# adityamwagh/SuperSLAM

Measured on AMD Instinct MI355X. Metric: stereo pairs/sec (SPx2+LG) at 1376x376, higher is better.
Workload: dtype f16; 1 GPU; configs[1]: SuperPoint x2 + select + gather + 1x LightGlue on 1376x376 stereo pairs; a step = 8 x 64 = 512 pairs per GPU resident in HBM (8 library calls of 64 pairs, different images per call), max_keypoints 600, seeded synthetic weights; pairs_per_call=64, max_keypoints=600, matches_last_call=1412, parallelism=replicated weights, pairs sharded over 1 rank(s), no data-path collective

## Files before the change

superslam_amd/csrc/lg_ffn.h:

```cpp
#pragma once
#include "igemm.h"
#include "kernels.h"

namespace sship {

constexpr int kFfnLd = 520;
typedef float f2_t __attribute__((ext_vector_type(2)));
constexpr float kGeluQ0 = -2.301893292e+00f, kGeluQ1 = -1.054467824e-01f, kGeluQ2 = 4.423903354e-04f, kGeluQ3 = 7.747288073e-05f,
                kGeluQ4 = -2.787147429e-06f;
__device__ __forceinline__ f2_t gelu2(f2_t y) {
  const f2_t s = y * y;
  f2_t q = s * kGeluQ4 + kGeluQ3;
  q = q * s + kGeluQ2;
  q = q * s + kGeluQ1;
  q = q * s + kGeluQ0;
  const f2_t t = y * q;
  const f2_t d = {1.0f + __builtin_amdgcn_exp2f(t[0]), 1.0f + __builtin_amdgcn_exp2f(t[1])};
  const f2_t r = {__builtin_amdgcn_rcpf(d[0]), __builtin_amdgcn_rcpf(d[1])};
  return y * r;
}
struct FfnTail {
  int ntiles;
  IgemmArgs proj;
  unsigned long long* trace;
  int trace_it;
  const float* match_w;
  float match_b;
  float* logsig;
  int n_main;
  const void* pf_ptr[3];
  int pf_bytes[3];
  const int* live;
  int tiles_per_pair;
};

bool ffn16_applicable(int tokens, int next_mt, bool heads);
hipError_t launch_lg_ffn16(int tokens, int next_mt, bool heads, hipStream_t s, const _Float16* ctx, const _Float16* w0p, const float* b0,
                           const float* gamma, const float* beta, const _Float16* w3p, const float* b3, _Float16* x, FfnTail t);

}
```

superslam_amd/csrc/lg_kernels.hip:

```cpp
#include <cstdlib>
#include <type_traits>

#include "igemm.h"
#include "kernels.h"
#include "lg_ffn.h"

namespace sship {

__global__ __launch_bounds__(256) void k_lg_prep(const float* __restrict__ kp, int kp_stride, int kp_seq_stride,
                                                 const int* __restrict__ lens, int max_kp, int* __restrict__ lens_clamped,
                                                 const _Float16* __restrict__ desc,
                                                 size_t desc_seq_stride, const float* __restrict__ wr, float img_w,
                                                 float img_h, int S, int NP, _Float16* __restrict__ x,
                                                 float* __restrict__ rope, float* __restrict__ kpn) {
  if (blockIdx.x == 0 && (int)threadIdx.x < S) lens_clamped[threadIdx.x] = min(max(lens[threadIdx.x], 0), max_kp);
  if (blockIdx.x == 0)
    for (int i = 256 + threadIdx.x; i < S; i += 256) lens_clamped[i] = min(max(lens[i], 0), max_kp);
  const int token = blockIdx.x * 4 + (threadIdx.x >> 6);
  const int lane = threadIdx.x & 63;
  if (token >= S * NP) return;
  const int s = token / NP, n = token % NP;
  const bool valid = n < min(max(lens[s], 0), max_kp);
  h4_t v = to_h4(0.f, 0.f, 0.f, 0.f);
  if (valid) v = *reinterpret_cast<const h4_t*>(desc + (size_t)s * desc_seq_stride + (size_t)n * 256 + lane * 4);
// ... 421 lines not shown
  } else {
    launch_attn<1, 4>(q, k, vt, lens, d, cross, ctx, s);
  }
}

#ifndef SSHIP_FFN_ABL
#define SSHIP_FFN_ABL 0
#endif
#ifndef SSHIP_FFN_DEEP_PFK
#define SSHIP_FFN_DEEP_PFK 4
#endif
#ifndef SSHIP_FFN_DEEP
#define SSHIP_FFN_DEEP 1
#endif
__device__ __forceinline__ void ffn_bar_lds() { asm volatile("s_waitcnt lgkmcnt(0)\n\ts_barrier" ::: "memory"); }
template <int AD>
__device__ __forceinline__ int ffn_live_tiles(const FfnTail& t) {
  if constexpr (AD == 1) return t.live[0] * t.tiles_per_pair;
  else if constexpr (AD == 2) return t.live[0];
  else return t.ntiles;
}
template <int AD>
__device__ __forceinline__ int ffn_tile_of(const FfnTail& t, int li) {
  if constexpr (AD == 1) return t.live[1 + li / t.tiles_per_pair] * t.tiles_per_pair + li % t.tiles_per_pair;
  else if constexpr (AD == 2) return t.live[1 + li];
  else return li;
}
template <int NEXT_MT, bool HEADS, int NT, bool PROJ, int AD = 0>
__global__ __launch_bounds__(512, 2) void k_lg_ffn(const _Float16* __restrict__ ctx, const _Float16* __restrict__ w0p,
                                                const float* __restrict__ b0, const float* __restrict__ gamma,
                                                const float* __restrict__ beta, const _Float16* __restrict__ w3p,
                                                const float* __restrict__ b3, _Float16* __restrict__ x, FfnTail tail) {
  constexpr int NTOK = NT * 32;
  constexpr bool DEEP = NT == 1 && !PROJ && SSHIP_FFN_DEEP;
  auto barrier = [&]() __attribute__((always_inline)) { if constexpr (DEEP) ffn_bar_lds(); else __syncthreads(); };
  constexpr int G0 = 4;
  constexpr int XBUF = NTOK * kFfnLd;
  extern __shared__ __attribute__((aligned(16))) char ffn_smem[];
  _Float16* s_xbuf = reinterpret_cast<_Float16*>(ffn_smem);
  float (*s_red)[NTOK] = reinterpret_cast<float (*)[NTOK]>(s_xbuf + (NT <= 2 ? 2 : 1) * XBUF);
  float* s_par = reinterpret_cast<float*>(s_red) + 16 * NTOK;
  for (int i = threadIdx.x; i < (PROJ ? 0 : 1792); i += 512)
    s_par[i] = i < 512 ? b0[i] : i < 1024 ? gamma[i - 512] : i < 1536 ? beta[i - 1024] : b3[i - 1536];
// ... 237 lines not shown
      const int rope_segs_t = pj.flags & 0xf;
      float4 cs[4][NT], bqk[NQK > 0 ? NQK : 1][4];
      if constexpr (HEADS) {
        if (rope_segs_t > 0) {
#pragma unroll
          for (int g = 0; g < 4; ++g)
#pragma unroll
            for (int n = 0; n < NT; ++n)
              cs[g][n] = *reinterpret_cast<const float4*>(pj.aux + (t0 + n * 32 + j) * 64 + ((wave * 32) & 63) + hh * 4 + g * 8 + zero);
        }
#pragma unroll
        for (int m = 0; m < NQK; ++m)
#pragma unroll
          for (int g = 0; g < 4; ++g) bqk[m][g] = *reinterpret_cast<const float4*>(pj.bias + (m * 8 + wave) * 32 + hh * 4 + g * 8);
      }
      constexpr int NG = (16 - PFK) / GT;
      h8_t at[2][GT][NEXT_MT];
      if constexpr (NG > 0) {
#pragma unroll
        for (int i = 0; i < GT; ++i)
#pragma unroll
          for (int m = 0; m < NEXT_MT; ++m) at[0][i][m] = *reinterpret_cast<const h8_t*>(wp + ((PFK + i) * NEXT_MT + m) * 512);
      }
      auto kstep = [&](int ks, const h8_t (&a)[NEXT_MT]) __attribute__((always_inline)) {
        h8_t bf[NT];
#pragma unroll
        for (int n = 0; n < NT; ++n) bf[n] = *reinterpret_cast<const h8_t*>(bfp + n * 32 * kFfnLd + ks * 16);
#pragma unroll
        for (int m = 0; m < NEXT_MT; ++m) {
#pragma unroll
// ... 71 lines not shown
                }
                const h2_t p01 = {(_Float16)v0, (_Float16)v1}, p23 = {(_Float16)v2, (_Float16)v3};
                lo[g] = __builtin_bit_cast(unsigned, p01);
                hi[g] = __builtin_bit_cast(unsigned, p23);
              }
#pragma unroll
              for (int gp = 0; gp < 2; ++gp) {
                const auto s0 = __builtin_amdgcn_permlane32_swap(lo[2 * gp], lo[2 * gp + 1], false, false);
                const auto s1 = __builtin_amdgcn_permlane32_swap(hi[2 * gp], hi[2 * gp + 1], false, false);
                const int u = ((R0 & 63) >> 3) + 2 * gp + hh;
                *reinterpret_cast<uint4*>(dst + (u >> 1) * 512 + (((u & 1) << 5) + j) * 8) = make_uint4(s0[0], s1[0], s0[1], s1[1]);
              }
            }
          }
        }
      } else {
        EpiF16<false, false>::template run<NEXT_MT, NT>(pj, ac3, 0, (int)(t0 >> 5), j, wave * NEXT_MT * 32, hh);
      }
    };
    if constexpr (HEADS) run_tail(std::integral_constant<int, 1 << (NEXT_MT - 1)>{});
    else run_tail(std::integral_constant<int, 0>{});
    if (tail.logsig) {
#pragma unroll 1
      for (int tk = wave * (NTOK / 8); tk < (wave + 1) * (NTOK / 8); ++tk) {
        const h4_t v = *reinterpret_cast<const h4_t*>(s_x + tk * kFfnLd + lane * 4);
        float d = 0.f;
#pragma unroll
        for (int e = 0; e < 4; ++e) d += (float)v[e] * mwq[lane * 4 + e];
        const float z = wave_sum(d) + tail.match_b;
        if (lane == 0) tail.logsig[t0 + tk] = fminf(z, 0.f) - log1pf(expf(-fabsf(z)));
      }
    }
  }
  stamp(9);
  if (NT > 2 && has_next) {
    __syncthreads();
    stage_tile(ffn_tile_of<AD>(tail, li + nwg), s_xn, wave, lane);
    asm volatile("s_waitcnt vmcnt(0)" ::: "memory");
  }
  if constexpr (PROJ) asm volatile("s_waitcnt vmcnt(0)" ::: "memory");
  if (has_next) __syncthreads();
  stamp(10);
  }
}
template <int NEXT_MT, bool HEADS, int NT, bool PROJ, int AD = 0, typename... A>
static hipError_t launch_ffn_nt(int tokens, int extra_wg, hipStream_t s, A... args) {
  constexpr size_t smem = (size_t)(NT <= 2 ? 2 : 1) * NT * 32 * kFfnLd * 2 + 16 * NT * 32 * 4 + 1792 * 4;
  static_assert(smem <= 163840, "LDS budget");
  auto kern = k_lg_ffn<NEXT_MT, HEADS, NT, PROJ, AD>;
  static const hipError_t attr_rc = hipFuncSetAttribute(reinterpret_cast<const void*>(kern), hipFuncAttributeMaxDynamicSharedMemorySize, (int)smem);
  if (attr_rc != hipSuccess) return attr_rc;
  const int ntiles = tokens / (NT * 32);
  hipLaunchKernelGGL(kern, dim3((ntiles < cu_count() ? ntiles : cu_count()) + extra_wg), dim3(512), smem, s, args...);
  return hipGetLastError();
}
static void ffn_trace_report(unsigned long long* dev, int nwg, int next_mt, hipStream_t s) {
  std::vector<unsigned long long> h((size_t)nwg * 8 * 12);
  (void)hipStreamSynchronize(s);
  (void)hipMemcpy(h.data(), dev, h.size() * 8, hipMemcpyDeviceToHost);
  static const char* names[10] = {"ffn.0", "LN stats", "DMA issue+GELU", "barrier", "ffn.3", "vmcnt+barrier+residual", "barrier", "tail MFMA", "tail epilogue", "end barrier"};
  double sum[10] = {0}; long cnt = 0;
  for (int w = 0; w < nwg * 8; ++w) {
    const unsigned long long* t = h.data() + (size_t)w * 12;
    if (!t[0] || !t[10]) continue;
    for (int i = 0; i < 10; ++i) sum[i] += (double)(t[i + 1] > t[i] ? t[i + 1] - t[i] : 0);
    ++cnt;
  }
  if (!cnt) return;
  fprintf(stderr, "[ffn trace next_mt=%d, %ld waves]", next_mt, cnt);
  double tot = 0;
  for (int i = 0; i < 10; ++i) { fprintf(stderr, " %s=%.0f", names[i], sum[i] / cnt); tot += sum[i] / cnt; }
  fprintf(stderr, " | tile=%.0f clk\n", tot);
}
template <int NEXT_MT, bool HEADS, int AD = 0, typename... A>
static hipError_t launch_ffn(int nt, int tokens, int extra_wg, hipStream_t s, A... args) {
  return nt == 1 ? launch_ffn_nt<NEXT_MT, HEADS, 1, false, AD>(tokens, extra_wg, s, args...)
                 : launch_ffn_nt<NEXT_MT, HEADS, 2, false, AD>(tokens, extra_wg, s, args...);
}
#ifndef SSHIP_FFN4_XROWS
#define SSHIP_FFN4_XROWS 1
#endif
#ifndef SSHIP_FFN4_BSTORE
#define SSHIP_FFN4_BSTORE 5
#endif
#ifndef SSHIP_FFN4_ABL
#define SSHIP_FFN4_ABL 0
#endif
__device__ __forceinline__ f16x_t mfma32_abl(h8_t a, h8_t b, f16x_t c) {
  if constexpr ((SSHIP_FFN4_ABL & 1) != 0) {
    asm volatile("" :: "v"(a), "v"(b));
    return c;
  } else {
    return mfma32(a, b, c);
  }
}
template <int NEXT_MT, bool HEADS, bool PROJ, int AD = 0>
__global__ __launch_bounds__(256, 2) void k_lg_ffn4(const _Float16* __restrict__ ctx, const _Float16* __restrict__ w0p,
                                                    const float* __restrict__ b0, const float* __restrict__ gamma,
                                                    const float* __restrict__ beta, const _Float16* __restrict__ w3p,
                                                    const float* __restrict__ b3, _Float16* __restrict__ x, FfnTail tail) {
  constexpr int NT = 2, NTOK = 64;
  extern __shared__ __attribute__((aligned(16))) char ffn_smem[];
  _Float16* s_x = reinterpret_cast<_Float16*>(ffn_smem);
  float (*s_red)[NTOK] = reinterpret_cast<float (*)[NTOK]>(s_x + NTOK * kFfnLd);
  float* s_par = reinterpret_cast<float*>(s_red) + 8 * NTOK;
  float* s_pb = s_par + 1792;
  float* s_b0b = s_pb + 768;
  for (int i = threadIdx.x; i < (PROJ ? 0 : 1792); i += 256)
    s_par[i] = i < 512 ? b0[i] : i < 1024 ? gamma[i - 512] : i < 1536 ? beta[i - 1024] : b3[i - 1536];
  for (int i = threadIdx.x; i < (PROJ ? 0 : 512); i += 256) s_b0b[i] = b0[i];
  if constexpr (NEXT_MT > 0 && HEADS)
    for (int i = threadIdx.x; i < NEXT_MT * 256; i += 256) s_pb[i] = tail.proj.bias[i];
  auto stage_tile = [&](int tile, int wave, int lane) {
    const size_t tt = (size_t)tile * NTOK;
    const char* gsrc = reinterpret_cast<const char*>((lane < 32 ? x + lane * 8 : ctx + (lane - 32) * 8) + (tt + wave) * 256);
#pragma unroll
    for (int k = 0; k < NTOK / 4; k += 2) {
      const unsigned lds0 = __builtin_amdgcn_readfirstlane((unsigned)(uintptr_t)(s_x + (wave + 4 * k) * kFfnLd));
      const unsigned lds1 = __builtin_amdgcn_readfirstlane((unsigned)(uintptr_t)(s_x + (wave + 4 * k + 4) * kFfnLd)) - 2048u;
      unsigned keep;
      asm volatile("s_mov_b32 %0, m0\n\ts_mov_b32 m0, %2\n\ts_nop 0\n\tglobal_load_lds_dwordx4 %1, off\n\t"
                   "s_mov_b32 m0, %3\n\ts_nop 0\n\tglobal_load_lds_dwordx4 %1, off offset:2048\n\ts_mov_b32 m0, %0"
                   : "=&s"(keep) : "v"(gsrc), "s"(lds0), "s"(lds1) : "memory");
      gsrc += 4096;
    }
  };
// ... 208 lines not shown
  stamp(6);
  }
  if constexpr (NEXT_MT > 0) {
    __syncthreads();
    stamp(7);
    if constexpr (SSHIP_FFN4_XROWS && !PROJ) {
#pragma unroll
      for (int r2 = 0; r2 < NTOK / 8; ++r2) {
        const int row = wave * (NTOK / 4) + 2 * r2 + hh;
        const uint4 u = *reinterpret_cast<const uint4*>(s_x + row * kFfnLd + j * 8);
        *reinterpret_cast<uint4*>(x + (t0 + row) * 256 + j * 8) = u;
      }
    }
    const int NP = pj.np, nt32 = NP >> 5;
    const int rope_segs = pj.flags & 0xf;
#pragma unroll 1
    for (int pass = 0; pass < 2; ++pass) {
      const int cb = wave + 4 * pass;
      f16x_t ac3[NEXT_MT][NT];
#pragma unroll
      for (int m = 0; m < NEXT_MT; ++m)
#pragma unroll
        for (int n = 0; n < NT; ++n)
#pragma unroll
          for (int r = 0; r < 16; ++r) ac3[m][n][r] = 0.f;
      float4 cs[4][NT];
      const __amdgpu_buffer_rsrc_t rrope = __builtin_amdgcn_make_buffer_rsrc(const_cast<float*>(tail.proj.aux), 0, (int)0x7ffffff0, 0x00020000);
      if constexpr (HEADS) {
        if (rope_segs > 0) {
#pragma unroll
// ... 92 lines not shown
                hi[g] = __builtin_bit_cast(unsigned, p23);
              }
#pragma unroll
              for (int gp = 0; gp < 2; ++gp) {
                const auto s0 = __builtin_amdgcn_permlane32_swap(lo[2 * gp], lo[2 * gp + 1], false, false);
                const auto s1 = __builtin_amdgcn_permlane32_swap(hi[2 * gp], hi[2 * gp + 1], false, false);
                if (SSHIP_FFN4_BSTORE & 4) wstore(rqk, lane16, dst + ((((R0 & 63) >> 3) + 2 * gp) >> 1) * 512, wq_t{s0[0], s1[0], s0[1], s1[1]});
                else {
                  const int u = ((R0 & 63) >> 3) + 2 * gp + hh;
                  *reinterpret_cast<uint4*>(static_cast<_Float16*>(seg == 0 ? pj.out0 : pj.out1) + dst + (u >> 1) * 512 + (((u & 1) << 5) + j) * 8) = make_uint4(s0[0], s1[0], s0[1], s1[1]);
                }
              }
            }
          }
        }
      } else {
        EpiF16<false, false>::template run<NEXT_MT, NT>(pj, ac3, 0, (int)(t0 >> 5), j, cb * NEXT_MT * 32, hh);
      }
    }
    if (tail.logsig) {
#pragma unroll 1
      for (int tk = wave * (NTOK / 4); tk < (wave + 1) * (NTOK / 4); ++tk) {
        const h4_t v = *reinterpret_cast<const h4_t*>(s_x + tk * kFfnLd + lane * 4);
        float d = 0.f;
#pragma unroll
        for (int e = 0; e < 4; ++e) d += (float)v[e] * mwq[lane * 4 + e];
        const float z = wave_sum(d) + tail.match_b;
        if (lane == 0) tail.logsig[t0 + tk] = fminf(z, 0.f) - log1pf(expf(-fabsf(z)));
      }
    }
  }
  stamp(10);
  if (has_next) {
    __syncthreads();
    stage_tile(ffn_tile_of<AD>(tail, li + (int)gridDim.x), wave, lane);
    asm volatile("s_waitcnt vmcnt(0)" ::: "memory");
    __syncthreads();
  }
  stamp(11);
  }
}
template <int NEXT_MT, bool HEADS, bool PROJ, int AD = 0, typename... A>
static hipError_t launch_ffn4(int tokens, hipStream_t s, A... args) {
  constexpr size_t smem = (size_t)64 * kFfnLd * 2 + 8 * 64 * 4 + (1792 + 768 + 512) * 4;
  static_assert(2 * smem <= 163840, "two workgroups must fit the CU's LDS");
  auto kern = k_lg_ffn4<NEXT_MT, HEADS, PROJ, AD>;
  static const hipError_t attr_rc = hipFuncSetAttribute(reinterpret_cast<const void*>(kern), hipFuncAttributeMaxDynamicSharedMemorySize, (int)smem);
  if (attr_rc != hipSuccess) return attr_rc;
  const int ntiles = tokens / 64;
  hipLaunchKernelGGL(kern, dim3(ntiles < 2 * cu_count() ? ntiles : 2 * cu_count()), dim3(256), smem, s, args...);
  return hipGetLastError();
}
static bool use_ffn4(int tokens) {
  static const int env = dev_env("SUPERSLAM_HIP_FFN") ? atoi(dev_env("SUPERSLAM_HIP_FFN")) : 0;
  if ((size_t)tokens * 512 >= 0x7f000000ull) return false;
  if (env == 8) return false;
  if (env == 4) return tokens % 64 == 0;
  return tokens % 64 == 0 && tokens / 64 >= 2 * cu_count();
}

[[maybe_unused]] static bool use_ffn16(int tokens) {
// ... 72 lines not shown
#if SSHIP_DEV_SWITCHES
  if (!live && use_ffn16(tokens) && ffn16_applicable(tokens, mt, heads)) {
    (void)launch_lg_ffn16(tokens, mt, heads, s, ctx, w0.w, w0.bias, gamma, beta, w3.w, w3.bias, x, t);
    return;
  }
#endif
  t.live = live;
  const int ad = live ? live_mode : 0;
  if (use_ffn4(tokens) && !trace_on_is8()) {
    t.ntiles = tokens / 64;
    t.tiles_per_pair = 2 * d.NP / 64;
    auto go4 = [&](auto ad_c) {
      constexpr int AD = decltype(ad_c)::value;
      if (heads && mt == 3) (void)launch_ffn4<3, true, false, AD>(tokens, s, ctx, w0.w, w0.bias, gamma, beta, w3.w, w3.bias, x, t);
      else if (heads && mt == 2) (void)launch_ffn4<2, true, false, AD>(tokens, s, ctx, w0.w, w0.bias, gamma, beta, w3.w, w3.bias, x, t);
      else (void)launch_ffn4<1, false, false, AD>(tokens, s, ctx, w0.w, w0.bias, gamma, beta, w3.w, w3.bias, x, t);
    };
    if (ad == 2) go4(std::integral_constant<int, 2>{});
    else if (ad == 1) go4(std::integral_constant<int, 1>{});
    else go4(std::integral_constant<int, 0>{});
    if (trace_on) ffn4_trace_report(trace_buf, t.ntiles < 2 * cu_count() ? t.ntiles : 2 * cu_count(), mt, s);
    return;
  }
  t.tiles_per_pair = 2 * d.NP / (nt * 32);
  const int extra = ffn_prefetch_setup(t, trace_wg, prefetch);
  auto go = [&](auto ad_c) {
    constexpr int AD = decltype(ad_c)::value;
    if (heads && mt == 3) (void)launch_ffn<3, true, AD>(nt, tokens, extra, s, ctx, w0.w, w0.bias, gamma, beta, w3.w, w3.bias, x, t);
    else if (heads && mt == 2) (void)launch_ffn<2, true, AD>(nt, tokens, extra, s, ctx, w0.w, w0.bias, gamma, beta, w3.w, w3.bias, x, t);
    else (void)launch_ffn<1, false, AD>(nt, tokens, extra, s, ctx, w0.w, w0.bias, gamma, beta, w3.w, w3.bias, x, t);
  };
  if (ad == 2) go(std::integral_constant<int, 2>{});
  else if (ad == 1) go(std::integral_constant<int, 1>{});
  else go(std::integral_constant<int, 0>{});
  if (trace_on) ffn_trace_report(trace_buf, trace_wg, mt, s);
}

hipError_t launch_lg_proj_heads(const ConvW& next, _Float16* x, LgDims d, int rope_segs, int t_seg, const float* rope, _Float16* q,
                                _Float16* k, _Float16* vt, hipStream_t s, const ConvW* const* prefetch, const int* tiles) {
  if (next.cout != 768) return hipErrorInvalidValue;
  const int tokens = d.S * d.NP;
  FfnTail t{};
  const int nt = tokens / 64 < cu_count() / 2 ? 1 : 2;
  t.ntiles = tokens / (nt * 32);
// ... 153 lines not shown
    ms = mutual ? expf(w[2 * NP + i]) : 0.f;
    mj = (mutual && ms > thr) ? j : -1;
  }
  matches0[(size_t)pair * max_kp + i] = mj;
  mscores0[(size_t)pair * max_kp + i] = ms;
}
#endif
constexpr float kLog2e = 1.44269504088896340736f;
__device__ __forceinline__ float fast_exp(float x) { return __builtin_amdgcn_exp2f(x * kLog2e); }
__device__ __forceinline__ void lse_merge(float& m, float& s, float m2, float s2) {
  const float M = fmaxf(m, m2);
  const float a = m > -INFINITY ? s * fast_exp(m - M) : 0.f, b = m2 > -INFINITY ? s2 * fast_exp(m2 - M) : 0.f;
  m = M; s = a + b;
}
constexpr int kAssignCh = 4;
__device__ __forceinline__ float fold_lse(const float2* p, int nparts, int NP) {
  float m = -INFINITY, s = 0.f;
  for (int k = 0; k < nparts; ++k) { const float2 v = p[(size_t)k * NP]; lse_merge(m, s, v.x, v.y); }
  return m + logf(s);
}
__device__ __forceinline__ void fold_argmax(const float2* p, int nparts, int NP, float& best, int& bi) {
  best = -INFINITY; bi = 0x7fffffff;
  for (int k = 0; k < nparts; ++k) {
    const float2 v = p[(size_t)k * NP];
    const int i = __float_as_int(v.y);
    if (v.x > best || (v.x == best && i < bi)) { best = v.x; bi = i; }
  }
}
template <int PASS>
__global__ __launch_bounds__(256, 2) void k_assign_stream(const _Float16* __restrict__ md, const float* __restrict__ logsig,
                                                       const int* __restrict__ lens, int NP, float* __restrict__ pcol,
                                                       float* __restrict__ prow, const float* __restrict__ pcol_in,
                                                       const float* __restrict__ prow_in) {
  constexpr int kChunkCols = (kMaxKp / 32 + kAssignCh - 1) / kAssignCh * 32;
  __shared__ __attribute__((aligned(16))) float s_lc[PASS ? kChunkCols : 4];
  __shared__ float s_lr[PASS ? 128 : 4];
  const int pair = blockIdx.y, wave = threadIdx.x >> 6, lane = threadIdx.x & 63, jl = lane & 31, hh = lane >> 5;
  const int NT = NP >> 5, ti = blockIdx.x * 4 + wave, i0 = ti * 32;
  const int n0 = min(max(lens[2 * pair], 0), NP), n1 = min(max(lens[2 * pair + 1], 0), NP);
  if ((int)blockIdx.x * 128 >= n0) return;
  const bool active = ti < NT && i0 < n0;
  const _Float16* A = md + ((size_t)(2 * pair) * NP + min(i0 + jl, NP - 1)) * 256 + hh * 8;
  const _Float16* Bm = md + (size_t)(2 * pair + 1) * NP * 256;
  h8_t fa[16];
#pragma unroll
  for (int ks = 0; ks < 16; ++ks) fa[ks] = *reinterpret_cast<const h8_t*>(A + ks * 16);
  const int my_i = i0 + jl;
  const int ro = 4 * hh;
  float c_i = 0.f, c_r[PASS ? 16 : 1];
  float rm = -INFINITY, rs = 0.f;
  int rj = 0x7fffffff;
  const int ntj_all = (n1 + 31) >> 5, per = (ntj_all + kAssignCh - 1) / kAssignCh;
  const int tj_lo = blockIdx.z * per, ntj = min(tj_lo + per, ntj_all);
  if (tj_lo >= ntj) return;
  const int jc0 = tj_lo * 32;
  if constexpr (PASS == 1) {
    const int nch = (ntj_all + per - 1) / max(per, 1), nrt = (n0 + 31) >> 5;
    if (threadIdx.x < 128) {
      const int i = blockIdx.x * 128 + threadIdx.x;
      s_lr[threadIdx.x] = i < n0 ? fold_lse(reinterpret_cast<const float2*>(prow_in) + (size_t)pair * kAssignCh * NP + i, nch, NP) : 0.f;
    }
    for (int j = threadIdx.x; j < (ntj - tj_lo) * 32; j += 256) {
      const int jj = jc0 + j;
      s_lc[j] = jj < n1 ? logsig[(size_t)(2 * pair + 1) * NP + jj] - fold_lse(reinterpret_cast<const float2*>(pcol_in) + (size_t)pair * NT * NP + jj, nrt, NP)
                        : 0.f;
    }
    __syncthreads();
    c_i = logsig[(size_t)(2 * pair) * NP + min(my_i, NP - 1)] - s_lr[wave * 32 + jl];
#pragma unroll
    for (int r = 0; r < 16; ++r) {
      const int il = (r & 3) + 8 * (r >> 2) + ro;
      c_r[r] = logsig[(size_t)(2 * pair) * NP + min(i0 + il, NP - 1)] - s_lr[wave * 32 + il];
    }
  }
  constexpr int kRowH = 264;
  __shared__ __attribute__((aligned(16))) _Float16 s_b[2][32 * kRowH];
  typedef unsigned stg_t __attribute__((ext_vector_type(4)));
  stg_t stg[4];
  auto fetch = [&](int tj) __attribute__((always_inline)) {
#pragma unroll
    for (int q = 0; q < 4; ++q) {
      const int u = threadIdx.x + 256 * q, row = u >> 5, unit = u & 31;
      stg[q] = *reinterpret_cast<const stg_t*>(Bm + (size_t)min(tj * 32 + row, NP - 1) * 256 + unit * 8);
    }
  };
  auto put = [&](int buf) __attribute__((always_inline)) {
#pragma unroll
    for (int q = 0; q < 4; ++q) {
      const int u = threadIdx.x + 256 * q, row = u >> 5, unit = u & 31;
      *reinterpret_cast<stg_t*>(&s_b[buf][row * kRowH + unit * 8]) = stg[q];
    }
  };
  fetch(tj_lo);
  put(0);
  __syncthreads();
  for (int tj = tj_lo; tj < ntj; ++tj) {
    const int j0 = tj * 32, buf = (tj - tj_lo) & 1;
    fetch(min(tj + 1, ntj - 1));
    const f16x_t zero16 = {0.f, 0.f, 0.f, 0.f, 0.f, 0.f, 0.f, 0.f, 0.f, 0.f, 0.f, 0.f, 0.f, 0.f, 0.f, 0.f};
    f16x_t ai = zero16, aj = zero16;
    if (active) {
      const _Float16* bt = &s_b[buf][jl * kRowH + hh * 8];
#pragma unroll
      for (int k = 0; k < 16; ++k) {
        const h8_t fbk = *reinterpret_cast<const h8_t*>(bt + k * 16);
        ai = mfma32(fbk, fa[k], ai);
        aj = mfma32(fa[k], fbk, aj);
// ... 45 lines not shown
#pragma unroll
      for (int g = 0; g < 4; ++g) {
        const int jb = j0 + 8 * g + ro;
        const float4 d4 = *reinterpret_cast<const float4*>(s_lc + jb - jc0);
        const float dv[4] = {d4.x, d4.y, d4.z, d4.w};
#pragma unroll
        for (int e = 0; e < 4; ++e) {
          const float v = fmaf(2.f, ai[4 * g + e], dv[e]);
          if (v > rm) { rm = v; rj = jb + e; }
        }
      }
      const float d_j = s_lc[my_j - jc0];
      float cv = -INFINITY;
      int ci = 0x7fffffff;
#pragma unroll
      for (int r = 0; r < 16; ++r) {
        const int i = i0 + (r & 3) + 8 * (r >> 2) + ro;
        const float v = fmaf(2.f, aj[r], c_r[r]);
        if (v > cv) { cv = v; ci = i; }
      }
      const float ov = __shfl_xor(cv, 32, 64);
      const int oi = __shfl_xor(ci, 32, 64);
      if (ov > cv || (ov == cv && oi < ci)) { cv = ov; ci = oi; }
      if (hh == 0 && my_j < n1)
        *reinterpret_cast<float2*>(pcol + (((size_t)pair * NT + ti) * NP + my_j) * 2) = make_float2(cv + d_j, __int_as_float(ci));
    }
  }
  float2* pr = reinterpret_cast<float2*>(prow) + ((size_t)pair * kAssignCh + blockIdx.z) * NP + my_i;
  if constexpr (PASS == 0) {
    lse_merge(rm, rs, __shfl_xor(rm, 32, 64), __shfl_xor(rs, 32, 64));
    if (hh == 0 && my_i < n0) *pr = make_float2(rm, rs);
  } else {
    const float ov = __shfl_xor(rm, 32, 64);
    const int oj = __shfl_xor(rj, 32, 64);
    if (ov > rm || (ov == rm && oj < rj)) { rm = ov; rj = oj; }
    if (hh == 0 && my_i < n0) *pr = make_float2(rm + c_i, __int_as_float(rj));
  }
}
__global__ __launch_bounds__(256) void k_assign_mutual(const float* __restrict__ pcol, const float* __restrict__ prow,
                                                       const int* __restrict__ lens, int NP, int max_kp, float thr,
                                                       int32_t* __restrict__ matches0, float* __restrict__ mscores0) {
  const int pair = blockIdx.y, i = blockIdx.x * blockDim.x + threadIdx.x;
  if (i >= max_kp) return;
  const int n0 = min(max(lens[2 * pair], 0), NP), n1 = min(max(lens[2 * pair + 1], 0), NP);
  const int NT = NP >> 5;
  int mj = -1;
  float ms = 0.f;
  if (i < n0 && n1 > 0) {
    const int ntj_all = (n1 + 31) >> 5, per = (ntj_all + kAssignCh - 1) / kAssignCh;
    float best, cbest;
    int j, ci;
    fold_argmax(reinterpret_cast<const float2*>(prow) + (size_t)pair * kAssignCh * NP + i, (ntj_all + per - 1) / max(per, 1), NP, best, j);
    if (j == 0x7fffffff) j = 0;
    bool mutual = false;
    if ((unsigned)j < (unsigned)n1) {
      fold_argmax(reinterpret_cast<const float2*>(pcol) + (size_t)pair * NT * NP + j, (n0 + 31) >> 5, NP, cbest, ci);
      mutual = (ci == 0x7fffffff ? 0 : ci) == i;
    }
    ms = mutual ? expf(best) : 0.f;
    mj = (mutual && ms > thr) ? j : -1;
  }
  matches0[(size_t)pair * max_kp + i] = mj;
  mscores0[(size_t)pair * max_kp + i] = ms;
}

void launch_lg_assign(const _Float16* md, const float* logsig, const int* lens, LgDims d, float* ws, float* pcol, int max_kp,
                      int32_t* matches0, float* mscores0, float thr, int stage, hipStream_t s) {
  const int P = d.S / 2, NT = d.NP / 32;
#if SSHIP_DEV_SWITCHES
  static const bool legacy = dev_env("SUPERSLAM_HIP_LG_ASSIGN") && std::string(dev_env("SUPERSLAM_HIP_LG_ASSIGN")) == "matrix";
  if (legacy && stage == 0) {
    float* sim = pcol;
    launch_lg_sim(md, lens, d, sim, s);
    hipLaunchKernelGGL(k_assign_row_lse, dim3(d.NP / 4, P), dim3(256), 0, s, sim, lens, d.NP, ws);
    hipLaunchKernelGGL(k_assign_col_lse, dim3((d.NP + 63) / 64, P), dim3(64 * kColRG), 0, s, sim, lens, d.NP, ws);
    hipLaunchKernelGGL(k_assign_row_arg, dim3(d.NP / 4, P), dim3(256), 0, s, sim, logsig, lens, d.NP, ws);
    hipLaunchKernelGGL(k_assign_col_arg, dim3((d.NP + 63) / 64, P), dim3(64 * kColRG), 0, s, sim, logsig, lens, d.NP, ws);
    hipLaunchKernelGGL(k_assign_final, dim3((max_kp + 255) / 256, P), dim3(256), 0, s, lens, d.NP, ws, max_kp, thr, matches0, mscores0);
    return;
  }
#endif
  {
    float* prow = pcol + (size_t)P * NT * d.NP * 2;
    float* pcol1 = prow + (size_t)P * kAssignCh * d.NP * 2;
    float* prow1 = pcol1 + (size_t)P * NT * d.NP * 2;
    if (stage == 0 || stage == 1)
      hipLaunchKernelGGL(k_assign_stream<0>, dim3((NT + 3) / 4, P, kAssignCh), dim3(256), 0, s, md, logsig, lens, d.NP, pcol, prow, nullptr, nullptr);
    if (stage == 0 || stage == 2)
      hipLaunchKernelGGL(k_assign_stream<1>, dim3((NT + 3) / 4, P, kAssignCh), dim3(256), 0, s, md, logsig, lens, d.NP, pcol1, prow1, pcol, prow);
    if (stage == 0)
      hipLaunchKernelGGL(k_assign_mutual, dim3((max_kp + 255) / 256, P), dim3(256), 0, s, pcol1, prow1, lens, d.NP, max_kp, thr, matches0, mscores0);
  }
}

__global__ __launch_bounds__(256) void k_lg_depth_init(const int* __restrict__ lens, int np, LgDepth dep) {
  for (int q = threadIdx.x; q < np; q += 256) {
    dep.layers_run[q] = 9;
#pragma unroll
    for (int i = 0; i < 8; ++i) dep.cnt[q * 8 + i] = 0;
    dep.lens_live[2 * q] = lens[2 * q];
    dep.lens_live[2 * q + 1] = lens[2 * q + 1];
    dep.live[1 + q] = q;
  }
  if (threadIdx.x == 0) { dep.live[0] = np; *dep.ticket = 0u; }
}
void launch_lg_depth_init(const int* lens, int np, LgDepth dep, hipStream_t s) {
// ... 303 lines not shown
```

Measured before the change: 5623 pairs/s.

## Stage final-projection output through LDS and batch assignment fold loads

The final LightGlue FFN projection epilogue now writes biased results into LDS, computes the match-head logsigmoid in-kernel, and then writes coalesced full rows of the descriptor output instead of using the generic epilogue. The assignment kernels batch the partial-LSE and argmax fold loads (B loads in flight before merging), keep per-row corrections in LDS rather than 16 registers, defer the A-fragment loads, and raise pass-1 occupancy to 3 workgroups. The old paths stay reachable through an env switch. The aim is fewer uncoalesced stores, more memory-level parallelism in the serial folds, and lower register pressure, at the cost of an extra barrier and more LDS traffic.

```diff
diff --git a/superslam_amd/csrc/lg_ffn.h b/superslam_amd/csrc/lg_ffn.h
--- a/superslam_amd/csrc/lg_ffn.h
+++ b/superslam_amd/csrc/lg_ffn.h
@@ -34,6 +34,49 @@
   int tiles_per_pair;
 };
 
+template <int NT>
+__device__ __forceinline__ void ffn_md_to_lds(_Float16* s_md, const f16x_t (&acc)[NT], const float4 (&bv)[4], int j, int hh, int c0) {
+#pragma unroll
+  for (int g = 0; g < 4; ++g)
+#pragma unroll
+    for (int n = 0; n < NT; ++n)
+      *reinterpret_cast<h4_t*>(s_md + (n * 32 + j) * kFfnLd + c0 + hh * 4 + g * 8) =
+          to_h4(acc[n][4 * g + 0] + bv[g].x, acc[n][4 * g + 1] + bv[g].y, acc[n][4 * g + 2] + bv[g].z, acc[n][4 * g + 3] + bv[g].w);
+}
+template <int NTOK, int NW>
+__device__ __forceinline__ void ffn_md_rows(const _Float16* s_md, _Float16* md_tile, int wave, int lane) {
+  const int j = lane & 31, hh = lane >> 5;
+#pragma unroll
+  for (int r2 = 0; r2 < NTOK / NW / 2; ++r2) {
+    const int row = wave * (NTOK / NW) + 2 * r2 + hh;
+    const uint4 u = *reinterpret_cast<const uint4*>(s_md + row * kFfnLd + j * 8);
+    *reinterpret_cast<uint4*>(md_tile + (size_t)row * 256 + j * 8) = u;
+  }
+}
+template <int TPW>
+__device__ __forceinline__ void ffn_match_head(const _Float16* s_x, float4 w4, float match_b, float* logsig_tile, int wave, int lane) {
+  static_assert(TPW <= 64, "one lane per token");
+  const float w[4] = {w4.x, w4.y, w4.z, w4.w};
+  float d[TPW];
+#pragma unroll
+  for (int t = 0; t < TPW; ++t) {
+    const h4_t v = *reinterpret_cast<const h4_t*>(s_x + (wave * TPW + t) * kFfnLd + lane * 4);
+    float a = 0.f;
+#pragma unroll
+    for (int e = 0; e < 4; ++e) a += (float)v[e] * w[e];
+    d[t] = a;
+  }
+#pragma unroll
+  for (int o = 32; o > 0; o >>= 1)
+#pragma unroll
+    for (int t = 0; t < TPW; ++t) d[t] += __shfl_xor(d[t], o, 64);
+  float z = d[0];
+#pragma unroll
+  for (int t = 1; t < TPW; ++t) z = lane == t ? d[t] : z;
+  z += match_b;
+  if (lane < TPW) logsig_tile[wave * TPW + lane] = fminf(z, 0.f) - log1pf(expf(-fabsf(z)));
+}
+
 bool ffn16_applicable(int tokens, int next_mt, bool heads);
 hipError_t launch_lg_ffn16(int tokens, int next_mt, bool heads, hipStream_t s, const _Float16* ctx, const _Float16* w0p, const float* b0,
                            const float* gamma, const float* beta, const _Float16* w3p, const float* b3, _Float16* x, FfnTail t);
diff --git a/superslam_amd/csrc/lg_kernels.hip b/superslam_amd/csrc/lg_kernels.hip
--- a/superslam_amd/csrc/lg_kernels.hip
+++ b/superslam_amd/csrc/lg_kernels.hip
@@ -459,6 +459,10 @@
 #define SSHIP_FFN_DEEP 1
 #endif
 __device__ __forceinline__ void ffn_bar_lds() { asm volatile("s_waitcnt lgkmcnt(0)\n\ts_barrier" ::: "memory"); }
+static bool lg_closing_serial() {
+  static const bool serial = dev_env("SUPERSLAM_HIP_LG_CLOSING") && std::string(dev_env("SUPERSLAM_HIP_LG_CLOSING")) == "serial";
+  return serial;
+}
 template <int AD>
 __device__ __forceinline__ int ffn_live_tiles(const FfnTail& t) {
   if constexpr (AD == 1) return t.live[0] * t.tiles_per_pair;
@@ -471,7 +475,7 @@
   else if constexpr (AD == 2) return t.live[1 + li];
   else return li;
 }
-template <int NEXT_MT, bool HEADS, int NT, bool PROJ, int AD = 0>
+template <int NEXT_MT, bool HEADS, int NT, bool PROJ, int AD = 0, bool OLDC = false>
 __global__ __launch_bounds__(512, 2) void k_lg_ffn(const _Float16* __restrict__ ctx, const _Float16* __restrict__ w0p,
                                                 const float* __restrict__ b0, const float* __restrict__ gamma,
                                                 const float* __restrict__ beta, const _Float16* __restrict__ w3p,
@@ -739,6 +743,12 @@
 #pragma unroll
           for (int g = 0; g < 4; ++g) bqk[m][g] = *reinterpret_cast<const float4*>(pj.bias + (m * 8 + wave) * 32 + hh * 4 + g * 8);
       }
+      float4 bfin[4], mw4 = make_float4(0.f, 0.f, 0.f, 0.f);
+      if constexpr (!HEADS && !OLDC) {
+#pragma unroll
+        for (int g = 0; g < 4; ++g) bfin[g] = *reinterpret_cast<const float4*>(pj.bias + wave * 32 + hh * 4 + g * 8);
+        if (tail.logsig) mw4 = *reinterpret_cast<const float4*>(mwq + lane * 4);
+      }
       constexpr int NG = (16 - PFK) / GT;
       h8_t at[2][GT][NEXT_MT];
       if constexpr (NG > 0) {
@@ -840,13 +850,19 @@
             }
           }
         }
+      } else if constexpr (OLDC) {
+        EpiF16<false, false>::template run<NEXT_MT, NT>(pj, ac3, 0, (int)(t0 >> 5), j, wave * NEXT_MT * 32, hh);
       } else {
-        EpiF16<false, false>::template run<NEXT_MT, NT>(pj, ac3, 0, (int)(t0 >> 5), j, wave * NEXT_MT * 32, hh);
+        static_assert(HEADS || NEXT_MT == 1, "final_proj has one M-tile per wave");
+        ffn_md_to_lds<NT>(s_x + 256, ac3[0], bfin, j, hh, wave * 32);
+        if (tail.logsig) ffn_match_head<NTOK / 8>(s_x, mw4, tail.match_b, tail.logsig + t0, wave, lane);
+        barrier();
+        ffn_md_rows<NTOK, 8>(s_x + 256, static_cast<_Float16*>(pj.out0) + t0 * 256, wave, lane);
       }
     };
     if constexpr (HEADS) run_tail(std::integral_constant<int, 1 << (NEXT_MT - 1)>{});
     else run_tail(std::integral_constant<int, 0>{});
-    if (tail.logsig) {
+    if (tail.logsig && (HEADS || OLDC)) {
 #pragma unroll 1
       for (int tk = wave * (NTOK / 8); tk < (wave + 1) * (NTOK / 8); ++tk) {
         const h4_t v = *reinterpret_cast<const h4_t*>(s_x + tk * kFfnLd + lane * 4);
@@ -869,11 +885,11 @@
   stamp(10);
   }
 }
-template <int NEXT_MT, bool HEADS, int NT, bool PROJ, int AD = 0, typename... A>
+template <int NEXT_MT, bool HEADS, int NT, bool PROJ, int AD = 0, bool OLDC = false, typename... A>
 static hipError_t launch_ffn_nt(int tokens, int extra_wg, hipStream_t s, A... args) {
   constexpr size_t smem = (size_t)(NT <= 2 ? 2 : 1) * NT * 32 * kFfnLd * 2 + 16 * NT * 32 * 4 + 1792 * 4;
   static_assert(smem <= 163840, "LDS budget");
-  auto kern = k_lg_ffn<NEXT_MT, HEADS, NT, PROJ, AD>;
+  auto kern = k_lg_ffn<NEXT_MT, HEADS, NT, PROJ, AD, OLDC>;
   static const hipError_t attr_rc = hipFuncSetAttribute(reinterpret_cast<const void*>(kern), hipFuncAttributeMaxDynamicSharedMemorySize, (int)smem);
   if (attr_rc != hipSuccess) return attr_rc;
   const int ntiles = tokens / (NT * 32);
@@ -898,10 +914,10 @@
   for (int i = 0; i < 10; ++i) { fprintf(stderr, " %s=%.0f", names[i], sum[i] / cnt); tot += sum[i] / cnt; }
   fprintf(stderr, " | tile=%.0f clk\n", tot);
 }
-template <int NEXT_MT, bool HEADS, int AD = 0, typename... A>
+template <int NEXT_MT, bool HEADS, int AD = 0, bool OLDC = false, typename... A>
 static hipError_t launch_ffn(int nt, int tokens, int extra_wg, hipStream_t s, A... args) {
-  return nt == 1 ? launch_ffn_nt<NEXT_MT, HEADS, 1, false, AD>(tokens, extra_wg, s, args...)
-                 : launch_ffn_nt<NEXT_MT, HEADS, 2, false, AD>(tokens, extra_wg, s, args...);
+  return nt == 1 ? launch_ffn_nt<NEXT_MT, HEADS, 1, false, AD, OLDC>(tokens, extra_wg, s, args...)
+                 : launch_ffn_nt<NEXT_MT, HEADS, 2, false, AD, OLDC>(tokens, extra_wg, s, args...);
 }
 #ifndef SSHIP_FFN4_XROWS
 #define SSHIP_FFN4_XROWS 1
@@ -920,7 +936,7 @@
     return mfma32(a, b, c);
   }
 }
-template <int NEXT_MT, bool HEADS, bool PROJ, int AD = 0>
+template <int NEXT_MT, bool HEADS, bool PROJ, int AD = 0, bool OLDC = false>
 __global__ __launch_bounds__(256, 2) void k_lg_ffn4(const _Float16* __restrict__ ctx, const _Float16* __restrict__ w0p,
                                                     const float* __restrict__ b0, const float* __restrict__ gamma,
                                                     const float* __restrict__ beta, const _Float16* __restrict__ w3p,
@@ -935,7 +951,7 @@
   for (int i = threadIdx.x; i < (PROJ ? 0 : 1792); i += 256)
     s_par[i] = i < 512 ? b0[i] : i < 1024 ? gamma[i - 512] : i < 1536 ? beta[i - 1024] : b3[i - 1536];
   for (int i = threadIdx.x; i < (PROJ ? 0 : 512); i += 256) s_b0b[i] = b0[i];
-  if constexpr (NEXT_MT > 0 && HEADS)
+  if constexpr (NEXT_MT > 0 && (HEADS || !OLDC))
     for (int i = threadIdx.x; i < NEXT_MT * 256; i += 256) s_pb[i] = tail.proj.bias[i];
   auto stage_tile = [&](int tile, int wave, int lane) {
     const size_t tt = (size_t)tile * NTOK;
@@ -1174,6 +1190,10 @@
     }
     const int NP = pj.np, nt32 = NP >> 5;
     const int rope_segs = pj.flags & 0xf;
+    float4 mw4 = make_float4(0.f, 0.f, 0.f, 0.f);
+    if constexpr (!HEADS && !OLDC) {
+      if (tail.logsig) mw4 = *reinterpret_cast<const float4*>(mwq + lane * 4);
+    }
 #pragma unroll 1
     for (int pass = 0; pass < 2; ++pass) {
       const int cb = wave + 4 * pass;
@@ -1296,11 +1316,21 @@
             }
           }
         }
+      } else if constexpr (OLDC) {
+        EpiF16<false, false>::template run<NEXT_MT, NT>(pj, ac3, 0, (int)(t0 >> 5), j, cb * NEXT_MT * 32, hh);
       } else {
-        EpiF16<false, false>::template run<NEXT_MT, NT>(pj, ac3, 0, (int)(t0 >> 5), j, cb * NEXT_MT * 32, hh);
-      }
-    }
-    if (tail.logsig) {
+        static_assert(HEADS || NEXT_MT == 1, "final_proj has one M-tile per block");
+        float4 bv[4];
+#pragma unroll
+        for (int g = 0; g < 4; ++g) bv[g] = *reinterpret_cast<const float4*>(s_pb + cb * 32 + hh * 4 + g * 8);
+        ffn_md_to_lds<NT>(s_x + 256, ac3[0], bv, j, hh, cb * 32);
+      }
+    }
+    if constexpr (!HEADS && !OLDC) {
+      if (tail.logsig) ffn_match_head<NTOK / 4>(s_x, mw4, tail.match_b, tail.logsig + t0, wave, lane);
+      __syncthreads();
+      ffn_md_rows<NTOK, 4>(s_x + 256, static_cast<_Float16*>(pj.out0) + t0 * 256, wave, lane);
+    } else if (tail.logsig) {
 #pragma unroll 1
       for (int tk = wave * (NTOK / 4); tk < (wave + 1) * (NTOK / 4); ++tk) {
         const h4_t v = *reinterpret_cast<const h4_t*>(s_x + tk * kFfnLd + lane * 4);
@@ -1322,11 +1352,11 @@
   stamp(11);
   }
 }
-template <int NEXT_MT, bool HEADS, bool PROJ, int AD = 0, typename... A>
+template <int NEXT_MT, bool HEADS, bool PROJ, int AD = 0, bool OLDC = false, typename... A>
 static hipError_t launch_ffn4(int tokens, hipStream_t s, A... args) {
   constexpr size_t smem = (size_t)64 * kFfnLd * 2 + 8 * 64 * 4 + (1792 + 768 + 512) * 4;
   static_assert(2 * smem <= 163840, "two workgroups must fit the CU's LDS");
-  auto kern = k_lg_ffn4<NEXT_MT, HEADS, PROJ, AD>;
+  auto kern = k_lg_ffn4<NEXT_MT, HEADS, PROJ, AD, OLDC>;
   static const hipError_t attr_rc = hipFuncSetAttribute(reinterpret_cast<const void*>(kern), hipFuncAttributeMaxDynamicSharedMemorySize, (int)smem);
   if (attr_rc != hipSuccess) return attr_rc;
   const int ntiles = tokens / 64;
@@ -1429,6 +1459,7 @@
       constexpr int AD = decltype(ad_c)::value;
       if (heads && mt == 3) (void)launch_ffn4<3, true, false, AD>(tokens, s, ctx, w0.w, w0.bias, gamma, beta, w3.w, w3.bias, x, t);
       else if (heads && mt == 2) (void)launch_ffn4<2, true, false, AD>(tokens, s, ctx, w0.w, w0.bias, gamma, beta, w3.w, w3.bias, x, t);
+      else if (lg_closing_serial()) (void)launch_ffn4<1, false, false, AD, SSHIP_DEV_SWITCHES != 0>(tokens, s, ctx, w0.w, w0.bias, gamma, beta, w3.w, w3.bias, x, t);
       else (void)launch_ffn4<1, false, false, AD>(tokens, s, ctx, w0.w, w0.bias, gamma, beta, w3.w, w3.bias, x, t);
     };
     if (ad == 2) go4(std::integral_constant<int, 2>{});
@@ -1443,6 +1474,7 @@
     constexpr int AD = decltype(ad_c)::value;
     if (heads && mt == 3) (void)launch_ffn<3, true, AD>(nt, tokens, extra, s, ctx, w0.w, w0.bias, gamma, beta, w3.w, w3.bias, x, t);
     else if (heads && mt == 2) (void)launch_ffn<2, true, AD>(nt, tokens, extra, s, ctx, w0.w, w0.bias, gamma, beta, w3.w, w3.bias, x, t);
+    else if (lg_closing_serial()) (void)launch_ffn<1, false, AD, SSHIP_DEV_SWITCHES != 0>(nt, tokens, extra, s, ctx, w0.w, w0.bias, gamma, beta, w3.w, w3.bias, x, t);
     else (void)launch_ffn<1, false, AD>(nt, tokens, extra, s, ctx, w0.w, w0.bias, gamma, beta, w3.w, w3.bias, x, t);
   };
   if (ad == 2) go(std::integral_constant<int, 2>{});
@@ -1626,27 +1658,55 @@
   m = M; s = a + b;
 }
 constexpr int kAssignCh = 4;
+constexpr int kFoldCols = 16;
+template <int B, bool SERIAL>
 __device__ __forceinline__ float fold_lse(const float2* p, int nparts, int NP) {
   float m = -INFINITY, s = 0.f;
-  for (int k = 0; k < nparts; ++k) { const float2 v = p[(size_t)k * NP]; lse_merge(m, s, v.x, v.y); }
+  if constexpr (SERIAL) {
+    for (int k = 0; k < nparts; ++k) { const float2 v = p[(size_t)k * NP]; lse_merge(m, s, v.x, v.y); }
+  } else {
+    for (int k0 = 0; k0 < nparts; k0 += B) {
+      f2_t v[B];
+#pragma unroll
+      for (int b = 0; b < B; ++b) v[b] = *reinterpret_cast<const f2_t*>(p + (size_t)min(k0 + b, nparts - 1) * NP);
+#pragma unroll
+      for (int b = 0; b < B; ++b)
+        if (k0 + b < nparts) lse_merge(m, s, v[b][0], v[b][1]);
+    }
+  }
   return m + logf(s);
 }
+template <int B, bool SERIAL>
 __device__ __forceinline__ void fold_argmax(const float2* p, int nparts, int NP, float& best, int& bi) {
   best = -INFINITY; bi = 0x7fffffff;
-  for (int k = 0; k < nparts; ++k) {
-    const float2 v = p[(size_t)k * NP];
+  auto take = [&](float2 v) __attribute__((always_inline)) {
     const int i = __float_as_int(v.y);
     if (v.x > best || (v.x == best && i < bi)) { best = v.x; bi = i; }
-  }
-}
-template <int PASS>
-__global__ __launch_bounds__(256, 2) void k_assign_stream(const _Float16* __restrict__ md, const float* __restrict__ logsig,
+  };
+  if constexpr (SERIAL) {
+    for (int k = 0; k < nparts; ++k) take(p[(size_t)k * NP]);
+  } else {
+    for (int k0 = 0; k0 < nparts; k0 += B) {
+      f2_t v[B];
+#pragma unroll
+      for (int b = 0; b < B; ++b) v[b] = *reinterpret_cast<const f2_t*>(p + (size_t)min(k0 + b, nparts - 1) * NP);
+#pragma unroll
+      for (int b = 0; b < B; ++b)
+        if (k0 + b < nparts) take(make_float2(v[b][0], v[b][1]));
+    }
+  }
+}
+#ifndef SSHIP_ASSIGN_P1_WGS
+#define SSHIP_ASSIGN_P1_WGS 3
+#endif
+template <int PASS, bool SERIAL = false>
+__global__ __launch_bounds__(256, PASS == 1 && !SERIAL ? SSHIP_ASSIGN_P1_WGS : 2) void k_assign_stream(const _Float16* __restrict__ md, const float* __restrict__ logsig,
                                                        const int* __restrict__ lens, int NP, float* __restrict__ pcol,
                                                        float* __restrict__ prow, const float* __restrict__ pcol_in,
                                                        const float* __restrict__ prow_in) {
   constexpr int kChunkCols = (kMaxKp / 32 + kAssignCh - 1) / kAssignCh * 32;
   __shared__ __attribute__((aligned(16))) float s_lc[PASS ? kChunkCols : 4];
-  __shared__ float s_lr[PASS ? 128 : 4];
+  __shared__ __attribute__((aligned(16))) float s_lr[PASS ? 128 : 4];
   const int pair = blockIdx.y, wave = threadIdx.x >> 6, lane = threadIdx.x & 63, jl = lane & 31, hh = lane >> 5;
   const int NT = NP >> 5, ti = blockIdx.x * 4 + wave, i0 = ti * 32;
   const int n0 = min(max(lens[2 * pair], 0), NP), n1 = min(max(lens[2 * pair + 1], 0), NP);
@@ -1654,12 +1714,10 @@
   const bool active = ti < NT && i0 < n0;
   const _Float16* A = md + ((size_t)(2 * pair) * NP + min(i0 + jl, NP - 1)) * 256 + hh * 8;
   const _Float16* Bm = md + (size_t)(2 * pair + 1) * NP * 256;
-  h8_t fa[16];
-#pragma unroll
-  for (int ks = 0; ks < 16; ++ks) fa[ks] = *reinterpret_cast<const h8_t*>(A + ks * 16);
   const int my_i = i0 + jl;
+  const int wave_s = __builtin_amdgcn_readfirstlane(wave);
   const int ro = 4 * hh;
-  float c_i = 0.f, c_r[PASS ? 16 : 1];
+  float c_i = 0.f, c_r[PASS && SERIAL ? 16 : 1];
   float rm = -INFINITY, rs = 0.f;
   int rj = 0x7fffffff;
   const int ntj_all = (n1 + 31) >> 5, per = (ntj_all + kAssignCh - 1) / kAssignCh;
@@ -1670,19 +1728,27 @@
     const int nch = (ntj_all + per - 1) / max(per, 1), nrt = (n0 + 31) >> 5;
     if (threadIdx.x < 128) {
       const int i = blockIdx.x * 128 + threadIdx.x;
-      s_lr[threadIdx.x] = i < n0 ? fold_lse(reinterpret_cast<const float2*>(prow_in) + (size_t)pair * kAssignCh * NP + i, nch, NP) : 0.f;
+      const float l0 = SERIAL ? 0.f : logsig[(size_t)(2 * pair) * NP + min(i, NP - 1)];
+      const float lse = i < n0 ? fold_lse<kAssignCh, SERIAL>(reinterpret_cast<const float2*>(prow_in) + (size_t)pair * kAssignCh * NP + i, nch, NP) : 0.f;
+      s_lr[threadIdx.x] = SERIAL ? lse : l0 - lse;
     }
     for (int j = threadIdx.x; j < (ntj - tj_lo) * 32; j += 256) {
       const int jj = jc0 + j;
-      s_lc[j] = jj < n1 ? logsig[(size_t)(2 * pair + 1) * NP + jj] - fold_lse(reinterpret_cast<const float2*>(pcol_in) + (size_t)pair * NT * NP + jj, nrt, NP)
-                        : 0.f;
+      float d = 0.f;
+      if (jj < n1) {
+        const float l1 = logsig[(size_t)(2 * pair + 1) * NP + jj];
+        d = l1 - fold_lse<kFoldCols, SERIAL>(reinterpret_cast<const float2*>(pcol_in) + (size_t)pair * NT * NP + jj, nrt, NP);
+      }
+      s_lc[j] = d;
     }
     __syncthreads();
-    c_i = logsig[(size_t)(2 * pair) * NP + min(my_i, NP - 1)] - s_lr[wave * 32 + jl];
-#pragma unroll
-    for (int r = 0; r < 16; ++r) {
-      const int il = (r & 3) + 8 * (r >> 2) + ro;
-      c_r[r] = logsig[(size_t)(2 * pair) * NP + min(i0 + il, NP - 1)] - s_lr[wave * 32 + il];
+    if constexpr (SERIAL) {
+      c_i = logsig[(size_t)(2 * pair) * NP + min(my_i, NP - 1)] - s_lr[wave * 32 + jl];
+#pragma unroll
+      for (int r = 0; r < 16; ++r) {
+        const int il = (r & 3) + 8 * (r >> 2) + ro;
+        c_r[r] = logsig[(size_t)(2 * pair) * NP + min(i0 + il, NP - 1)] - s_lr[wave * 32 + il];
+      }
     }
   }
   constexpr int kRowH = 264;
@@ -1703,6 +1769,9 @@
       *reinterpret_cast<stg_t*>(&s_b[buf][row * kRowH + unit * 8]) = stg[q];
     }
   };
+  h8_t fa[16];
+#pragma unroll
+  for (int ks = 0; ks < 16; ++ks) fa[ks] = *reinterpret_cast<const h8_t*>(A + ks * 16);
   fetch(tj_lo);
   put(0);
   __syncthreads();
@@ -1778,10 +1847,21 @@
       float cv = -INFINITY;
       int ci = 0x7fffffff;
 #pragma unroll
-      for (int r = 0; r < 16; ++r) {
-        const int i = i0 + (r & 3) + 8 * (r >> 2) + ro;
-        const float v = fmaf(2.f, aj[r], c_r[r]);
-        if (v > cv) { cv = v; ci = i; }
+      for (int g = 0; g < 4; ++g) {
+        float c4[4];
+        if constexpr (SERIAL) {
+#pragma unroll
+          for (int e = 0; e < 4; ++e) c4[e] = c_r[PASS && SERIAL ? 4 * g + e : 0];
+        } else {
+          const float4 t = *reinterpret_cast<const float4*>(s_lr + wave * 32 + 8 * g + ro);
+          c4[0] = t.x; c4[1] = t.y; c4[2] = t.z; c4[3] = t.w;
+        }
+#pragma unroll
+        for (int e = 0; e < 4; ++e) {
+          const int i = i0 + 8 * g + ro + e;
+          const float v = fmaf(2.f, aj[4 * g + e], c4[e]);
+          if (v > cv) { cv = v; ci = i; }
+        }
       }
       const float ov = __shfl_xor(cv, 32, 64);
       const int oi = __shfl_xor(ci, 32, 64);
@@ -1790,17 +1870,27 @@
         *reinterpret_cast<float2*>(pcol + (((size_t)pair * NT + ti) * NP + my_j) * 2) = make_float2(cv + d_j, __int_as_float(ci));
     }
   }
-  float2* pr = reinterpret_cast<float2*>(prow) + ((size_t)pair * kAssignCh + blockIdx.z) * NP + my_i;
-  if constexpr (PASS == 0) {
-    lse_merge(rm, rs, __shfl_xor(rm, 32, 64), __shfl_xor(rs, 32, 64));
-    if (hh == 0 && my_i < n0) *pr = make_float2(rm, rs);
+  if constexpr (PASS == 0 || SERIAL) {
+    float2* pr = reinterpret_cast<float2*>(prow) + ((size_t)pair * kAssignCh + blockIdx.z) * NP + my_i;
+    if constexpr (PASS == 0) {
+      lse_merge(rm, rs, __shfl_xor(rm, 32, 64), __shfl_xor(rs, 32, 64));
+      if (hh == 0 && my_i < n0) *pr = make_float2(rm, rs);
+    } else {
+      const float ov = __shfl_xor(rm, 32, 64);
+      const int oj = __shfl_xor(rj, 32, 64);
+      if (ov > rm || (ov == rm && oj < rj)) { rm = ov; rj = oj; }
+      if (hh == 0 && my_i < n0) *pr = make_float2(rm + c_i, __int_as_float(rj));
+    }
   } else {
+    const int ln = __lane_id(), row = wave_s * 32 + (ln & 31), i = blockIdx.x * 128 + row;
     const float ov = __shfl_xor(rm, 32, 64);
     const int oj = __shfl_xor(rj, 32, 64);
     if (ov > rm || (ov == rm && oj < rj)) { rm = ov; rj = oj; }
-    if (hh == 0 && my_i < n0) *pr = make_float2(rm + c_i, __int_as_float(rj));
-  }
-}
+    if ((ln & 32) == 0 && i < n0)
+      *(reinterpret_cast<float2*>(prow) + ((size_t)pair * kAssignCh + blockIdx.z) * NP + i) = make_float2(rm + s_lr[row], __int_as_float(rj));
+  }
+}
+template <bool SERIAL = false>
 __global__ __launch_bounds__(256) void k_assign_mutual(const float* __restrict__ pcol, const float* __restrict__ prow,
                                                        const int* __restrict__ lens, int NP, int max_kp, float thr,
                                                        int32_t* __restrict__ matches0, float* __restrict__ mscores0) {
@@ -1814,11 +1904,11 @@
     const int ntj_all = (n1 + 31) >> 5, per = (ntj_all + kAssignCh - 1) / kAssignCh;
     float best, cbest;
     int j, ci;
-    fold_argmax(reinterpret_cast<const float2*>(prow) + (size_t)pair * kAssignCh * NP + i, (ntj_all + per - 1) / max(per, 1), NP, best, j);
+    fold_argmax<kAssignCh, SERIAL>(reinterpret_cast<const float2*>(prow) + (size_t)pair * kAssignCh * NP + i, (ntj_all + per - 1) / max(per, 1), NP, best, j);
     if (j == 0x7fffffff) j = 0;
     bool mutual = false;
     if ((unsigned)j < (unsigned)n1) {
-      fold_argmax(reinterpret_cast<const float2*>(pcol) + (size_t)pair * NT * NP + j, (n0 + 31) >> 5, NP, cbest, ci);
+      fold_argmax<kFoldCols, SERIAL>(reinterpret_cast<const float2*>(pcol) + (size_t)pair * NT * NP + j, (n0 + 31) >> 5, NP, cbest, ci);
       mutual = (ci == 0x7fffffff ? 0 : ci) == i;
     }
     ms = mutual ? expf(best) : 0.f;
@@ -1848,12 +1938,16 @@
     float* prow = pcol + (size_t)P * NT * d.NP * 2;
     float* pcol1 = prow + (size_t)P * kAssignCh * d.NP * 2;
     float* prow1 = pcol1 + (size_t)P * NT * d.NP * 2;
+    constexpr bool kDev = SSHIP_DEV_SWITCHES != 0;
+    const bool serial = lg_closing_serial();
+    const auto pass1 = serial ? k_assign_stream<1, kDev> : k_assign_stream<1, false>;
+    const auto mutual = serial ? k_assign_mutual<kDev> : k_assign_mutual<false>;
     if (stage == 0 || stage == 1)
       hipLaunchKernelGGL(k_assign_stream<0>, dim3((NT + 3) / 4, P, kAssignCh), dim3(256), 0, s, md, logsig, lens, d.NP, pcol, prow, nullptr, nullptr);
     if (stage == 0 || stage == 2)
-      hipLaunchKernelGGL(k_assign_stream<1>, dim3((NT + 3) / 4, P, kAssignCh), dim3(256), 0, s, md, logsig, lens, d.NP, pcol1, prow1, pcol, prow);
+      hipLaunchKernelGGL(pass1, dim3((NT + 3) / 4, P, kAssignCh), dim3(256), 0, s, md, logsig, lens, d.NP, pcol1, prow1, pcol, prow);
     if (stage == 0)
-      hipLaunchKernelGGL(k_assign_mutual, dim3((max_kp + 255) / 256, P), dim3(256), 0, s, pcol1, prow1, lens, d.NP, max_kp, thr, matches0, mscores0);
+      hipLaunchKernelGGL(mutual, dim3((max_kp + 255) / 256, P), dim3(256), 0, s, pcol1, prow1, lens, d.NP, max_kp, thr, matches0, mscores0);
   }
 }
 
```

Result: no change. 5661 pairs/s (median of 6 runs) (+0.7%).
